# CleanDiffuserTeam/CleanDiffuser

Hardware: NVIDIA B200
Metric: sampled trajectories/sec (H=32, 100 DDPM steps) (higher is better)
Workload: dtype tf32 (fp32 activations and weights in HBM, tcgen05 kind::tf32, f32 accumulate)

## Files before the change

### __graft_entry__.py

```python
import os
import subprocess
import sys

ROOT = os.path.dirname(os.path.abspath(__file__))
CSRC = os.path.join(ROOT, "cleandiffuser_b200", "csrc")
LIB = os.path.join(CSRC, "libcds.so")
TC_PARTS = 8
HEADERS = ["common.cuh", "conv_simt.cuh", "conv_tc.cuh", "conv_ps.cuh", "ptx_sm100.cuh", "elementwise.cuh", "attention.cuh",
           os.path.join(ROOT, "include", "cds.h")]
OBJ_DIR = os.path.join(CSRC, "build")

NVCC_FLAGS = ["-gencode", "arch=compute_100a,code=sm_100a", "-O3", "-lineinfo", "-std=c++17",
              "-Xcompiler", "-fPIC", "-I" + os.path.join(ROOT, "include")]


def _units():
    units = [(os.path.join(OBJ_DIR, "cds_api.o"), os.path.join(CSRC, "cds_api.cu"), [])]
    for tf32 in (0, 1):
        for k in range(TC_PARTS):
            units.append((os.path.join(OBJ_DIR, f"conv_tc_inst_{k}_{'tf32' if tf32 else 'bf16'}.o"),
                          os.path.join(CSRC, "conv_tc_inst.cu"),
                          [f"-DCDS_TC_PART={k}", f"-DCDS_TC_PARTS={TC_PARTS}", f"-DCDS_TC_TF32={tf32}"]))
    units.append((os.path.join(OBJ_DIR, "conv_ps_inst.o"), os.path.join(CSRC, "conv_ps_inst.cu"), []))
    return units


def _newest_dep():
    deps = [f if os.path.isabs(f) else os.path.join(CSRC, f) for f in HEADERS]
    deps += [os.path.join(CSRC, f) for f in os.listdir(CSRC) if f.endswith((".cu", ".cuh"))]
    return max(os.path.getmtime(d) for d in deps if os.path.exists(d))


def build(force: bool = False) -> None:
    from concurrent.futures import ThreadPoolExecutor
    nvcc = os.environ.get("NVCC", "/usr/local/cuda/bin/nvcc")
    os.makedirs(OBJ_DIR, exist_ok=True)
    newest = _newest_dep()
    todo = [u for u in _units() if force or not os.path.exists(u[0]) or os.path.getmtime(u[0]) < newest]

    def compile_one(u):
        cmd = [nvcc] + NVCC_FLAGS + u[2] + ["-c", u[1], "-o", u[0]]
        print("[build]", " ".join(cmd), flush=True)
        r = subprocess.run(cmd, cwd=CSRC, capture_output=True, text=True)
        return u[0], r.returncode, r.stdout + r.stderr

    if todo:
        with ThreadPoolExecutor(max_workers=min(len(todo), os.cpu_count() or 1)) as ex:
            results = list(ex.map(compile_one, todo))
        for obj, rc, out in results:
            if rc != 0:
                raise RuntimeError(f"nvcc failed for {obj}:\n{out}")
    objs = [u[0] for u in _units()]
    if todo or not os.path.exists(LIB) or os.path.getmtime(LIB) < max(os.path.getmtime(o) for o in objs):
        cmd = [nvcc, "-gencode", "arch=compute_100a,code=sm_100a", "-shared", "-Xcompiler", "-fPIC"] + objs + ["-o", LIB]
        print("[build]", " ".join(cmd), flush=True)
        subprocess.run(cmd, check=True, cwd=CSRC)
    if ROOT not in sys.path:
        sys.path.insert(0, ROOT)
    import cleandiffuser_b200
    from cleandiffuser_b200.engine import cabi
    import ctypes
    lib = ctypes.CDLL(cabi.lib_path())
    missing = [s for s in cabi.EXPORTS if not hasattr(lib, s)]
    if missing:
        raise RuntimeError(f"libcds.so lacks symbols {missing}")
    print("[build] ok:", cabi.lib_path(), flush=True)


def smoke() -> None:
    if ROOT not in sys.path:
        sys.path.insert(0, ROOT)
    import torch
    from cleandiffuser_b200.diffusion import DiscreteDiffusionSDE
    from cleandiffuser_b200.engine import runtime
    from cleandiffuser_b200.nn_diffusion import JannerUNet1d
    from cleandiffuser_b200.testing import NoiseTape, load_synth
    import oracle.nets as onets
    import oracle.sampler as osamp

    assert torch.cuda.is_available(), "smoke() needs a CUDA device"
    os.environ["CDS_BACKEND"] = "cuda"
    dev = "cuda:0"
    B, H, D, T = 64, 32, 14, 10
    net = load_synth(JannerUNet1d(D, model_dim=32, emb_dim=32, kernel_size=5, dim_mult=[1, 2, 2, 2]), seed=0)
    sd = {k: v.clone() for k, v in net.state_dict().items()}
    mask = torch.zeros(H, D)
    mask[0, :11] = 1.
    agent = DiscreteDiffusionSDE(net, None, fix_mask=mask, predict_noise=False, diffusion_steps=T, device=dev)
    g = torch.Generator().manual_seed(1)
    prior = torch.zeros(B, H, D)
    prior[:, 0, :11] = torch.randn(B, 11, generator=g)

    fn = lambda x, t, c=None: onets.janner_unet(sd, x, t, c, emb_dim=32, kernel_size=5, n_stages=4)
    x_ref = None
    for math, tol_max, tol_mean in (("tf32", 2e-2, 2e-3), ("bf16", 0.2, 0.02), ("fp32", 2e-3, 2e-3)):
        os.environ["CDS_MATH"] = math
        before = runtime.STATS["engine_calls"]
        tape = NoiseTape() if x_ref is None else NoiseTape(tape.draws)
        with tape.active(), torch.no_grad():
            x_gpu, _ = agent.sample(prior.to(dev), solver="ddpm", n_samples=B, sample_steps=T, temperature=0.5)
        torch.cuda.synchronize()
        assert runtime.STATS["engine_calls"] == before + 1, "the CUDA engine did not run"
        if x_ref is None:
            with torch.no_grad():
                x_ref = osamp.sample_discrete(fn, prior, osamp.Tape([z.cpu().numpy() for z in tape.draws]), T=T, steps=T,
                                              solver="ddpm", temperature=0.5, fix_mask=mask[None], predict_noise=False)
        err = (x_gpu.cpu() - x_ref).abs()
        print(f"[smoke] JannerUNet1d B={B} H={H} d={D} DDPM {T} steps, math={math}: max|engine - oracle| = {err.max().item():.3e}, "
              f"mean = {err.mean().item():.3e}, launches={runtime.STATS['launches']}")
        assert err.max().item() < tol_max and err.mean().item() < tol_mean, (math, err.max().item(), err.mean().item())


if __name__ == "__main__":
    build()
    if len(sys.argv) > 1 and sys.argv[1] == "smoke":
        smoke()
```

### cleandiffuser_b200/csrc/cds_api.cu

```cuda
#include <cuda_runtime.h>

#include <cstdarg>
#include <cstdio>
#include <cstring>
#include <string>
#include <vector>

#include "cds.h"
#include "attention.cuh"
#include "conv_simt.cuh"
#include "conv_tc.cuh"
#include "conv_ps.cuh"
#include "attention_tma.cuh"
#include "linear_ln.cuh"
#include "elementwise.cuh"

namespace {

thread_local std::string g_err;

int fail(int code, const char* fmt, ...) {
  char buf[512];
  va_list ap;
  va_start(ap, fmt);
  vsnprintf(buf, sizeof buf, fmt, ap);
  va_end(ap);
  g_err = buf;
  return code;
}

#define CDS_CUDA(call)                                                                                  \
  do {                                                                                                  \
    cudaError_t e__ = (call);                                                                           \
    if (e__ != cudaSuccess) return fail(CDS_ERR_CUDA, "%s failed: %s", #call, cudaGetErrorString(e__)); \
  } while (0)

struct DeviceGuard {
  int prev = -1;
  cudaError_t err = cudaSuccess;
  explicit DeviceGuard(int device) {
    err = cudaGetDevice(&prev);
    if (err == cudaSuccess && prev != device) err = cudaSetDevice(device);
    else if (err == cudaSuccess) prev = -1;
  }
  ~DeviceGuard() { if (prev >= 0) cudaSetDevice(prev); }
};
#define CDS_ON_DEVICE(dev)                                                                                       \
  DeviceGuard guard__(dev);                                                                                      \
  if (guard__.err != cudaSuccess) return fail(CDS_ERR_CUDA, "cudaSetDevice(%d) failed: %s", (int)(dev), cudaGetErrorString(guard__.err))

struct Step {
  cds_op op;
  int conv_bn = 0;
  bool tc = false;
  cds::ConvTcLaunch tcl;
  int branch = 0;
  bool skip = false;
  bool ps = false;
  cds::ConvPsLaunch psl;
  cds::AttnTmaLaunch attl;
  bool fuse_ln = false;
  bool fused_into_prev = false;
  cds::LinLnLaunch lll;
};

int elementwise_grid(int64_t total, int sm_count) {
  int64_t blocks = (total + 255) / 256;
  int64_t cap = (int64_t)sm_count * 8;
  return (int)(blocks < cap ? (blocks > 0 ? blocks : 1) : cap);
}

int validate(const cds_op& op, Step* out) {
  out->op = op;
  out->branch = (op.flags & CDS_OPF_BRANCH_MASK) >> CDS_OPF_BRANCH_SHIFT;
  switch (op.kind) {
    case CDS_OP_CONV: {
      const cds_conv_op& c = op.u.conv;
      if (c.batch <= 0 || c.L_in <= 0 || c.L_out <= 0 || c.C_in <= 0 || c.C_out <= 0 || c.taps <= 0 ||
          c.stride <= 0 || c.phases <= 0)
        return fail(CDS_ERR_INVALID, "conv: non-positive geometry");
      if (!c.in || !c.w || !c.out) return fail(CDS_ERR_INVALID, "conv: null in/w/out");
      if (c.groups > 8) return fail(CDS_ERR_UNSUPPORTED, "conv: more than 8 GroupNorm groups");
      if (c.groups > 0 && (!c.gn_gamma || !c.gn_beta)) return fail(CDS_ERR_INVALID, "conv: GroupNorm without affine");
      if (c.res_w && (!c.res_in || c.res_C <= 0)) return fail(CDS_ERR_INVALID, "conv: shortcut conv without input");
      if (c.res_w && (c.stride != 1 || c.phases != 1)) return fail(CDS_ERR_INVALID, "conv: shortcut conv needs stride 1");
      if (c.math == CDS_MATH_BF16_TC || c.math == CDS_MATH_TF32_TC) {
        if (!cds::conv_tc_eligible(c))
          return fail(CDS_ERR_INVALID, "conv: op is not eligible for the tensor-core kernel (ask cds_conv_tc_supported)");
        if (cds::conv_ps_eligible(c)) {
          if (!cds::conv_ps_prepare(c, &out->psl))
            return fail(CDS_ERR_CUDA, "conv: cuTensorMapEncodeTiled failed (position-sliced, C_in=%d C_out=%d)", c.C_in, c.C_out);
          out->tc = out->ps = true;
          return CDS_OK;
        }
        if (!cds::conv_tc_prepare(c, &out->tcl))
          return fail(CDS_ERR_CUDA, "conv: cuTensorMapEncodeTiled failed (C_in=%d L=%d C_out=%d)", c.C_in, c.L_in, c.C_out);
        out->tc = true;
        return CDS_OK;
      }
      if (c.math != CDS_MATH_FP32) return fail(CDS_ERR_UNSUPPORTED, "conv: math mode %d unknown", c.math);
      if (c.sample_row_div > 1) return fail(CDS_ERR_UNSUPPORTED, "conv: sample_row_div needs the tensor-core kernel");
      out->conv_bn = cds::conv_simt_pick_bn(c);
      if (out->conv_bn == 0)
        return fail(CDS_ERR_UNSUPPORTED, "conv: GroupNorm tile does not fit (L_out=%d C_out=%d groups=%d)", c.L_out,
                    c.C_out, c.groups);
      return CDS_OK;
    }
    case CDS_OP_UPDATE: {
      const cds_update_op& u = op.u.update;
      if (u.batch <= 0 || u.row <= 0 || !u.x || !u.pred || !u.coef) return fail(CDS_ERR_INVALID, "update: bad arguments");
      if (u.mask && !u.prior) return fail(CDS_ERR_INVALID, "update: mask without prior");
      if (u.aux && !u.xhat_prev) return fail(CDS_ERR_INVALID, "update: aux history without xhat_prev");
      if (u.x_cast && (u.cast_C_in <= 0 || u.cast_C_out < u.cast_C_in || u.row % u.cast_C_in != 0))
        return fail(CDS_ERR_INVALID, "update: bad x_cast geometry");
      return CDS_OK;
    }
    case CDS_OP_LNMOD: {
      const cds_lnmod_op& l = op.u.lnmod;
      if (l.batch <= 0 || l.L <= 0 || l.C <= 0 || !l.in || !l.out || !l.shift || !l.scale)
        return fail(CDS_ERR_INVALID, "lnmod: bad arguments");
      return CDS_OK;
    }
    case CDS_OP_ATTN: {
      const cds_attn_op& a = op.u.attn;
      if (a.batch <= 0 || a.L <= 0 || a.heads <= 0 || a.C % a.heads != 0 || !a.qkv || !a.out)
        return fail(CDS_ERR_INVALID, "attn: bad arguments");
      int hd = a.C / a.heads;
      if (hd != 16 && hd != 32 && hd != 64) return fail(CDS_ERR_UNSUPPORTED, "attn: head_dim %d", hd);
      if ((size_t)a.L * hd * 8 > 200 * 1024) return fail(CDS_ERR_UNSUPPORTED, "attn: L=%d too long", a.L);
      if (a.qkv_dtype == CDS_BF16 && (hd != 32 || a.L > cds::kAttnMaxL || a.C % 8 != 0 || ((uintptr_t)a.qkv % 16) != 0))
        return fail(CDS_ERR_UNSUPPORTED, "attn: bf16 q/k/v needs head_dim 32, L <= %d, 16-byte aligned rows", cds::kAttnMaxL);
      if (cds::attention_tma_eligible(a) && !cds::attention_tma_prepare(a, &out->attl))
        return fail(CDS_ERR_CUDA, "attn: cuTensorMapEncodeTiled failed (L=%d C=%d)", a.L, a.C);
      return CDS_OK;
    }
    case CDS_OP_PREP: {
      const cds_prep_op& p = op.u.prep;
      if (p.batch <= 0 || p.row <= 0 || !p.x || !p.xin || !p.coef) return fail(CDS_ERR_INVALID, "prep: bad arguments");
      return CDS_OK;
    }
    case CDS_OP_CAST: {
      const cds_cast_op& k = op.u.cast;
      if (k.batch <= 0 || k.L <= 0 || k.C_in <= 0 || k.C_out < k.C_in || (k.C_out & 1) || !k.in || !k.out ||
          (k.out_dtype != CDS_F32 && k.out_dtype != CDS_BF16 && k.out_dtype != CDS_TF32))
        return fail(CDS_ERR_INVALID, "cast: bad arguments");
      return CDS_OK;
    }
    default:
      return fail(CDS_ERR_INVALID, "unknown operator kind %d", op.kind);
  }
}

int launch(const Step& s, const int* iter_ptr, int sm_count, cudaStream_t st, int* advance = nullptr, bool fused = false) {
  switch (s.op.kind) {
    case CDS_OP_CONV:
      if (fused && s.fuse_ln) CDS_CUDA(cds::linear_ln_launch(s.lll, iter_ptr, sm_count, st));
      else if (s.ps) CDS_CUDA(cds::conv_ps_launch(s.psl, iter_ptr, st));
      else if (s.tc) CDS_CUDA(cds::conv_tc_launch(s.tcl, iter_ptr, st));
      else CDS_CUDA(cds::conv_simt_launch(s.op.u.conv, s.conv_bn, iter_ptr, st));
      return CDS_OK;
    case CDS_OP_UPDATE: {
      const cds_update_op& u = s.op.u.update;
      cds::solver_update_kernel<<<elementwise_grid((int64_t)u.batch * u.row, sm_count), 256, 0, st>>>(u, iter_ptr, advance);
      CDS_CUDA(cudaGetLastError());
      return CDS_OK;
    }
    case CDS_OP_PREP: {
      const cds_prep_op& p = s.op.u.prep;
      cds::cm_prep_kernel<<<elementwise_grid((int64_t)p.batch * p.row, sm_count), 256, 0, st>>>(p, iter_ptr);
      CDS_CUDA(cudaGetLastError());
      return CDS_OK;
    }
    case CDS_OP_LNMOD: {
      const cds_lnmod_op& l = s.op.u.lnmod;
      int64_t rows = (int64_t)l.batch * l.L;
      int64_t blocks = (rows + 7) / 8;
      int64_t cap = (int64_t)sm_count * 8;
      cds::ln_modulate_kernel<<<(int)(blocks < cap ? blocks : cap), 256, 0, st>>>(l);
      CDS_CUDA(cudaGetLastError());
      return CDS_OK;
    }
    case CDS_OP_ATTN:
      if (s.attl.ok) CDS_CUDA(cds::attention_tma_launch(s.op.u.attn, s.attl, sm_count, st));
      else CDS_CUDA(cds::attention_launch(s.op.u.attn, st));
      return CDS_OK;
    case CDS_OP_CAST: {
      const cds_cast_op& k = s.op.u.cast;
      cds::cast_pad_kernel<<<elementwise_grid((int64_t)k.batch * k.L * (k.C_out / 2), sm_count), 256, 0, st>>>(k);
      CDS_CUDA(cudaGetLastError());
      return CDS_OK;
    }
  }
  return fail(CDS_ERR_INVALID, "unknown operator kind");
}

int preload_kernels() {
  cudaFuncAttributes a;
  CDS_CUDA(cudaFuncGetAttributes(&a, cds::conv_gemm_f32_kernel<32>));
  CDS_CUDA(cudaFuncGetAttributes(&a, cds::conv_gemm_f32_kernel<64>));
  CDS_CUDA(cudaFuncGetAttributes(&a, cds::conv_gemm_f32_kernel<128>));
  CDS_CUDA(cds::conv_tc_preload_all());
  CDS_CUDA(cds::conv_ps_preload_all());
  CDS_CUDA(cudaFuncGetAttributes(&a, cds::attention_f32_kernel<16>));
  CDS_CUDA(cudaFuncGetAttributes(&a, cds::attention_f32_kernel<32>));
  CDS_CUDA(cudaFuncGetAttributes(&a, cds::attention_f32_kernel<64>));
  CDS_CUDA(cudaFuncGetAttributes(&a, cds::attention_mma_hd32_kernel));
  CDS_CUDA(cudaFuncGetAttributes(&a, cds::attention_mma_tf32_hd32_kernel));
  CDS_CUDA(cds::attention_tma_preload_all());
  CDS_CUDA(cds::linear_ln_preload_all());
  CDS_CUDA(cudaFuncGetAttributes(&a, cds::solver_update_kernel));
  CDS_CUDA(cudaFuncGetAttributes(&a, cds::cm_prep_kernel));
  CDS_CUDA(cudaFuncGetAttributes(&a, cds::cast_pad_kernel));
  CDS_CUDA(cudaFuncGetAttributes(&a, cds::ln_modulate_kernel));
  CDS_CUDA(cudaFuncGetAttributes(&a, cds::set_iter_kernel));
  CDS_CUDA(cudaFuncGetAttributes(&a, cds::advance_iter_kernel));
  return CDS_OK;
}

}

namespace cds {
static long long* g_trace_buf = nullptr;
static int64_t g_trace_cap = 0;
static int g_trace_target = -1, g_trace_count = 0, g_trace_grid = 0;
long long* conv_tc_trace_hook(int grid) {
  if (!g_trace_buf) return nullptr;
  const int ord = g_trace_count++;
  if (ord != g_trace_target || (int64_t)grid * kTraceSlots > g_trace_cap) return nullptr;
  g_trace_grid = grid;
  return g_trace_buf;
}
}

struct cds_plan {
  int device = 0;
  int sm_count = 0;
  int n_iters = 0;
  bool finalized = false;
  std::vector<Step> steps;
  int* d_iter = nullptr;
  cudaStream_t cap_stream = nullptr;
  cudaGraph_t graph = nullptr;
  cudaGraphExec_t exec = nullptr;
  int multi = 0;
  int n_branches = 1;
  std::vector<cudaStream_t> side;
  cudaEvent_t ev_fork = nullptr;
  std::vector<cudaEvent_t> ev_join;
  cudaGraph_t graph_multi = nullptr;
  cudaGraphExec_t exec_multi = nullptr;
};

extern "C" {

int cds_version(void) { return CDS_ABI_VERSION; }
int cds_op_size(void) { return (int)sizeof(cds_op); }
const char* cds_last_error(void) { return g_err.c_str(); }

int cds_conv_tc_supported(const cds_conv_op* op) {
  if (!op) return 0;
  cds_conv_op c = *op;
  if (c.math != CDS_MATH_TF32_TC) c.math = CDS_MATH_BF16_TC;
  return cds::conv_tc_eligible(c) ? 1 : 0;
}

int cds_device_sm_count(int device) {
  int n = 0;
  if (cudaDeviceGetAttribute(&n, cudaDevAttrMultiProcessorCount, device) != cudaSuccess) return -1;
  return n;
}

int cds_plan_create(int device, cds_plan** out) {
  if (!out) return fail(CDS_ERR_INVALID, "plan_create: null out");
  int n_dev = 0;
  CDS_CUDA(cudaGetDeviceCount(&n_dev));
  if (device < 0 || device >= n_dev) return fail(CDS_ERR_INVALID, "plan_create: device %d of %d", device, n_dev);
  cds_plan* p = new cds_plan();
  p->device = device;
  p->sm_count = cds_device_sm_count(device);
  *out = p;
  return CDS_OK;
}

int cds_plan_destroy(cds_plan* p) {
  if (!p) return CDS_OK;
  DeviceGuard guard(p->device);
  if (p->exec) cudaGraphExecDestroy(p->exec);
  if (p->graph) cudaGraphDestroy(p->graph);
  if (p->exec_multi) cudaGraphExecDestroy(p->exec_multi);
  if (p->graph_multi) cudaGraphDestroy(p->graph_multi);
  if (p->cap_stream) cudaStreamDestroy(p->cap_stream);
  for (cudaStream_t s : p->side) cudaStreamDestroy(s);
  if (p->ev_fork) cudaEventDestroy(p->ev_fork);
  for (cudaEvent_t e : p->ev_join) cudaEventDestroy(e);
  if (p->d_iter) cudaFree(p->d_iter);
  delete p;
  return CDS_OK;
}

int cds_plan_append(cds_plan* p, const cds_op* ops, int32_t n_ops) {
  if (!p || (!ops && n_ops > 0)) return fail(CDS_ERR_INVALID, "plan_append: null argument");
  if (p->finalized) return fail(CDS_ERR_STATE, "plan_append after finalize");
  for (int i = 0; i < n_ops; ++i) {
    Step s;
    int rc = validate(ops[i], &s);
    if (rc != CDS_OK) {
      std::string inner = g_err;
      return fail(rc, "op %d: %s", (int)p->steps.size(), inner.c_str());
    }
    p->steps.push_back(s);
  }
  return CDS_OK;
}

int cds_plan_finalize(cds_plan* p, int32_t n_iters) {
  if (!p) return fail(CDS_ERR_INVALID, "plan_finalize: null plan");
  if (p->finalized) return fail(CDS_ERR_STATE, "plan already finalized");
  if (n_iters <= 0 || p->steps.empty()) return fail(CDS_ERR_INVALID, "plan_finalize: empty program");
  CDS_ON_DEVICE(p->device);
  { int rc = preload_kernels(); if (rc != CDS_OK) return rc; }
  CDS_CUDA(cudaMalloc(&p->d_iter, 2 * sizeof(int)));
  CDS_CUDA(cudaMemset(p->d_iter, 0, 2 * sizeof(int)));
  CDS_CUDA(cudaStreamCreateWithFlags(&p->cap_stream, cudaStreamNonBlocking));
  p->n_iters = n_iters;
  for (const Step& s : p->steps) if (s.branch + 1 > p->n_branches) p->n_branches = s.branch + 1;
  if (p->n_branches > 1) {
    CDS_CUDA(cudaEventCreateWithFlags(&p->ev_fork, cudaEventDisableTiming));
    for (int b = 1; b < p->n_branches; ++b) {
      cudaStream_t s; cudaEvent_t e;
      CDS_CUDA(cudaStreamCreateWithFlags(&s, cudaStreamNonBlocking));
      CDS_CUDA(cudaEventCreateWithFlags(&e, cudaEventDisableTiming));
      p->side.push_back(s); p->ev_join.push_back(e);
    }
    for (Step& s : p->steps) if (s.tc && !s.ps) s.tcl.max_ctas_per_sm = 1;
  }
  if (p->n_branches == 1) {
    for (size_t i = 0; i + 1 < p->steps.size(); ++i) {
      Step& a = p->steps[i];
      Step& b = p->steps[i + 1];
      if (a.op.kind != CDS_OP_CONV || b.op.kind != CDS_OP_LNMOD || !a.tc || a.ps) continue;
      if ((a.op.flags & CDS_OPF_ONCE) || (b.op.flags & CDS_OPF_ONCE)) continue;
      if (!cds::linear_ln_eligible(a.op.u.conv, b.op.u.lnmod)) continue;
      if (!cds::linear_ln_prepare(a.op.u.conv, b.op.u.lnmod, &a.lll)) continue;
      a.fuse_ln = true;
      b.fused_into_prev = true;
    }
  }
  p->finalized = true;
  return CDS_OK;
}

static bool advance_fused(const cds_plan* p) {
  if (p->n_branches > 1) return false;
  for (int i = (int)p->steps.size() - 1; i >= 0; --i)
    if (!(p->steps[i].op.flags & CDS_OPF_ONCE)) return p->steps[i].op.kind == CDS_OP_UPDATE;
  return false;
}

static int enqueue_once(cds_plan* p, cudaStream_t st) {
  for (const Step& s : p->steps) {
    if (!(s.op.flags & CDS_OPF_ONCE)) continue;
    int rc = launch(s, p->d_iter, p->sm_count, st);
    if (rc != CDS_OK) return rc;
  }
  return CDS_OK;
}

static int enqueue_iteration(cds_plan* p, cudaStream_t st) {
  const bool fused = advance_fused(p);
  if (p->n_branches == 1) {
    int last = -1;
    for (int i = 0; i < (int)p->steps.size(); ++i) if (!(p->steps[i].op.flags & CDS_OPF_ONCE)) last = i;
    for (int i = 0; i < (int)p->steps.size(); ++i) {
      const Step& s = p->steps[i];
      if ((s.op.flags & CDS_OPF_ONCE) || s.skip || s.fused_into_prev) continue;
      int rc = launch(s, p->d_iter, p->sm_count, st, (fused && i == last) ? p->d_iter : nullptr, true);
      if (rc != CDS_OK) return rc;
    }
  } else {
    CDS_CUDA(cudaEventRecord(p->ev_fork, st));
    for (cudaStream_t s : p->side) CDS_CUDA(cudaStreamWaitEvent(s, p->ev_fork, 0));
    std::vector<std::vector<int>> per(p->n_branches);
    for (int i = 0; i < (int)p->steps.size(); ++i) {
      const Step& s = p->steps[i];
      if (!(s.op.flags & CDS_OPF_ONCE) && !s.skip) per[s.branch].push_back(i);
    }
    for (size_t k = 0;; ++k) {
      bool any = false;
      for (int b = 0; b < p->n_branches; ++b) {
        if (k >= per[b].size()) continue;
        any = true;
        int rc = launch(p->steps[per[b][k]], p->d_iter, p->sm_count, b == 0 ? st : p->side[b - 1], nullptr);
        if (rc != CDS_OK) return rc;
      }
      if (!any) break;
    }
    for (int b = 1; b < p->n_branches; ++b) {
      CDS_CUDA(cudaEventRecord(p->ev_join[b - 1], p->side[b - 1]));
      CDS_CUDA(cudaStreamWaitEvent(st, p->ev_join[b - 1], 0));
    }
  }
  if (!fused) {
    cds::advance_iter_kernel<<<1, 1, 0, st>>>(p->d_iter);
    CDS_CUDA(cudaGetLastError());
  }
  return CDS_OK;
}

int cds_plan_run(cds_plan* p, int32_t first, int32_t count, void* stream, int32_t use_graph) {
  if (!p || !p->finalized) return fail(CDS_ERR_STATE, "plan_run before finalize");
  if (first < 0 || count < 0 || first + count > p->n_iters)
    return fail(CDS_ERR_INVALID, "plan_run: iterations [%d, %d) outside [0, %d)", first, first + count, p->n_iters);
  cudaStream_t st = reinterpret_cast<cudaStream_t>(stream);
  CDS_ON_DEVICE(p->device);
  if (use_graph && !p->exec) {
    CDS_CUDA(cudaStreamBeginCapture(p->cap_stream, cudaStreamCaptureModeThreadLocal));
    int rc = enqueue_iteration(p, p->cap_stream);
    cudaError_t e = cudaStreamEndCapture(p->cap_stream, &p->graph);
    if (rc != CDS_OK) return rc;
    if (e != cudaSuccess) return fail(CDS_ERR_CUDA, "graph capture failed: %s", cudaGetErrorString(e));
    CDS_CUDA(cudaGraphInstantiate(&p->exec, p->graph, 0));
    const char* gi = getenv("CDS_GRAPH_ITERS");
    p->multi = gi ? atoi(gi) : 10;
    if (p->multi > 1 && p->multi <= p->n_iters) {
      CDS_CUDA(cudaStreamBeginCapture(p->cap_stream, cudaStreamCaptureModeThreadLocal));
      int rc2 = CDS_OK;
      for (int k = 0; k < p->multi && rc2 == CDS_OK; ++k) rc2 = enqueue_iteration(p, p->cap_stream);
      cudaError_t e2 = cudaStreamEndCapture(p->cap_stream, &p->graph_multi);
      if (rc2 != CDS_OK) return rc2;
      if (e2 != cudaSuccess) return fail(CDS_ERR_CUDA, "graph capture (x%d) failed: %s", p->multi, cudaGetErrorString(e2));
      CDS_CUDA(cudaGraphInstantiate(&p->exec_multi, p->graph_multi, 0));
    } else {
      p->multi = 0;
    }
  }
  cds::set_iter_kernel<<<1, 1, 0, st>>>(p->d_iter, first);
  CDS_CUDA(cudaGetLastError());
  { int rc = enqueue_once(p, st); if (rc != CDS_OK) return rc; }
  for (int i = 0; i < count; ++i) {
    if (use_graph && p->exec_multi && count - i >= p->multi) {
      CDS_CUDA(cudaGraphLaunch(p->exec_multi, st));
      i += p->multi - 1;
    } else if (use_graph) {
      CDS_CUDA(cudaGraphLaunch(p->exec, st));
    } else {
      int rc = enqueue_iteration(p, st);
      if (rc != CDS_OK) return rc;
    }
  }
  return CDS_OK;
}

int cds_plan_run_range(cds_plan* p, int32_t iter, int32_t op_first, int32_t op_count, void* stream) {
  if (!p || !p->finalized) return fail(CDS_ERR_STATE, "plan_run_range before finalize");
  if (iter < 0 || iter >= p->n_iters) return fail(CDS_ERR_INVALID, "plan_run_range: iteration %d outside [0, %d)", iter, p->n_iters);
  if (op_first < 0 || op_count < 0 || op_first + op_count > (int)p->steps.size())
    return fail(CDS_ERR_INVALID, "plan_run_range: operators [%d, %d) outside [0, %d)", op_first, op_first + op_count, (int)p->steps.size());
  if (p->n_branches > 1) return fail(CDS_ERR_UNSUPPORTED, "plan_run_range: programs with parallel branches run whole iterations only");
  cudaStream_t st = reinterpret_cast<cudaStream_t>(stream);
  CDS_ON_DEVICE(p->device);
  cds::set_iter_kernel<<<1, 1, 0, st>>>(p->d_iter, iter);
  CDS_CUDA(cudaGetLastError());
  for (int i = op_first; i < op_first + op_count; ++i) {
    const Step& s = p->steps[i];
    if ((s.op.flags & CDS_OPF_ONCE) || s.skip) continue;
    if (s.fused_into_prev && i > op_first) continue;
    const bool both = s.fuse_ln && i + 1 < op_first + op_count;
    int rc = launch(s, p->d_iter, p->sm_count, st, nullptr, both);
    if (rc != CDS_OK) return rc;
  }
  return CDS_OK;
}

int cds_plan_profile(cds_plan* p, int32_t iter, void* stream, float* ms_per_op, int32_t n_ops) {
  if (!p || !p->finalized) return fail(CDS_ERR_STATE, "plan_profile before finalize");
  if (!ms_per_op || n_ops != (int)p->steps.size()) return fail(CDS_ERR_INVALID, "plan_profile: n_ops != %d", (int)p->steps.size());
  if (iter < 0 || iter >= p->n_iters) return fail(CDS_ERR_INVALID, "plan_profile: bad iteration");
  cudaStream_t st = reinterpret_cast<cudaStream_t>(stream);
  CDS_ON_DEVICE(p->device);
  std::vector<cudaEvent_t> ev(2 * n_ops);
  for (auto& e : ev) CDS_CUDA(cudaEventCreate(&e));
  cds::set_iter_kernel<<<1, 1, 0, st>>>(p->d_iter, iter);
  for (int pass = 0; pass < 2; ++pass) {
    for (int i = 0; i < n_ops; ++i) {
      const bool once = (p->steps[i].op.flags & CDS_OPF_ONCE) != 0;
      if (once != (pass == 0)) continue;
      CDS_CUDA(cudaEventRecord(ev[2 * i], st));
      if (!p->steps[i].skip && !p->steps[i].fused_into_prev) {
        int rc = launch(p->steps[i], p->d_iter, p->sm_count, st, nullptr, true);
        if (rc != CDS_OK) return rc;
      }
      CDS_CUDA(cudaEventRecord(ev[2 * i + 1], st));
    }
  }
  CDS_CUDA(cudaStreamSynchronize(st));
  for (int i = 0; i < n_ops; ++i) CDS_CUDA(cudaEventElapsedTime(&ms_per_op[i], ev[2 * i], ev[2 * i + 1]));
  for (auto& e : ev) cudaEventDestroy(e);
  return CDS_OK;
}

int cds_plan_launches_per_iter(const cds_plan* p) {
  if (!p) return 0;
  int n = advance_fused(p) ? 0 : 1;
  for (const Step& s : p->steps) if (!(s.op.flags & CDS_OPF_ONCE) && !s.skip && !s.fused_into_prev) ++n;
  return n;
}

int cds_debug_trace(void* device_buffer, int64_t capacity_entries, int32_t target_launch) {
  cds::g_trace_buf = reinterpret_cast<long long*>(device_buffer);
  cds::g_trace_cap = capacity_entries;
  cds::g_trace_target = target_launch;
  cds::g_trace_count = 0;
  int g = cds::g_trace_grid;
  cds::g_trace_grid = 0;
  return g;
}

int cds_run_op(int device, const cds_op* op, int32_t iter, void* stream) {
  if (!op) return fail(CDS_ERR_INVALID, "run_op: null op");
  CDS_ON_DEVICE(device);
  Step s;
  int rc = validate(*op, &s);
  if (rc != CDS_OK) return rc;
  cudaStream_t st = reinterpret_cast<cudaStream_t>(stream);
  int* d_iter = nullptr;
  CDS_CUDA(cudaMallocAsync(&d_iter, sizeof(int), st));
  cds::set_iter_kernel<<<1, 1, 0, st>>>(d_iter, iter);
  rc = launch(s, d_iter, cds_device_sm_count(device), st);
  cudaFreeAsync(d_iter, st);
  return rc;
}

}
```

Measured before the change: 67880.

## Fuse both tensor-core convolutions of a residual block into one persistent kernel

Adds a warp-specialized tcgen05 kernel that runs conv1+GroupNorm+Mish, keeps the hidden activation in shared memory, then runs conv2+GroupNorm+Mish plus the identity or 1x1-conv residual, all in one launch. The plan finalizer pairs consecutive TC conv steps when the intermediate buffer is read by no other step. The aim is to cut one launch per residual block and the HBM round trip of the intermediate. In exchange it adds a large new kernel with its own smem/TMEM planning and a more complex pipeline. It can be turned off with CDS_FUSE_RESBLOCK=0.

```diff
diff --git a/__graft_entry__.py b/__graft_entry__.py
--- a/__graft_entry__.py
+++ b/__graft_entry__.py
@@ -6,7 +6,7 @@
 CSRC = os.path.join(ROOT, "cleandiffuser_b200", "csrc")
 LIB = os.path.join(CSRC, "libcds.so")
 TC_PARTS = 8
-HEADERS = ["common.cuh", "conv_simt.cuh", "conv_tc.cuh", "conv_ps.cuh", "ptx_sm100.cuh", "elementwise.cuh", "attention.cuh",
+HEADERS = ["common.cuh", "conv_simt.cuh", "conv_tc.cuh", "conv_ps.cuh", "resblock_tc.cuh", "ptx_sm100.cuh", "elementwise.cuh", "attention.cuh",
            os.path.join(ROOT, "include", "cds.h")]
 OBJ_DIR = os.path.join(CSRC, "build")
 
@@ -22,6 +22,7 @@
                           os.path.join(CSRC, "conv_tc_inst.cu"),
                           [f"-DCDS_TC_PART={k}", f"-DCDS_TC_PARTS={TC_PARTS}", f"-DCDS_TC_TF32={tf32}"]))
     units.append((os.path.join(OBJ_DIR, "conv_ps_inst.o"), os.path.join(CSRC, "conv_ps_inst.cu"), []))
+    units.append((os.path.join(OBJ_DIR, "resblock_tc_inst.o"), os.path.join(CSRC, "resblock_tc_inst.cu"), []))
     return units
 
 
diff --git a/cleandiffuser_b200/csrc/cds_api.cu b/cleandiffuser_b200/csrc/cds_api.cu
--- a/cleandiffuser_b200/csrc/cds_api.cu
+++ b/cleandiffuser_b200/csrc/cds_api.cu
@@ -13,6 +13,7 @@
 #include "conv_ps.cuh"
 #include "attention_tma.cuh"
 #include "linear_ln.cuh"
+#include "resblock_tc.cuh"
 #include "elementwise.cuh"
 
 namespace {
@@ -62,7 +63,24 @@
   bool fuse_ln = false;
   bool fused_into_prev = false;
   cds::LinLnLaunch lll;
+  bool fuse_rb = false;
+  cds::ResblockLaunch rbl;
 };
+
+bool step_reads(const Step& s, const void* lo, const void* hi) {
+  auto in = [&](const void* q) { return q && q >= lo && q < hi; };
+  const cds_op& o = s.op;
+  switch (o.kind) {
+    case CDS_OP_CONV: return in(o.u.conv.in) || in(o.u.conv.res) || in(o.u.conv.res_in);
+    case CDS_OP_UPDATE: return in(o.u.update.x) || in(o.u.update.pred) || in(o.u.update.pred_uncond) || in(o.u.update.prior) ||
+                               in(o.u.update.xhat_prev) || in(o.u.update.aux);
+    case CDS_OP_LNMOD: return in(o.u.lnmod.in);
+    case CDS_OP_ATTN: return in(o.u.attn.qkv);
+    case CDS_OP_PREP: return in(o.u.prep.x);
+    case CDS_OP_CAST: return in(o.u.cast.in);
+  }
+  return true;
+}
 
 int elementwise_grid(int64_t total, int sm_count) {
   int64_t blocks = (total + 255) / 256;
@@ -155,6 +173,7 @@
   switch (s.op.kind) {
     case CDS_OP_CONV:
       if (fused && s.fuse_ln) CDS_CUDA(cds::linear_ln_launch(s.lll, iter_ptr, sm_count, st));
+      else if (fused && s.fuse_rb) CDS_CUDA(cds::resblock_launch(s.rbl, iter_ptr, sm_count, st));
       else if (s.ps) CDS_CUDA(cds::conv_ps_launch(s.psl, iter_ptr, st));
       else if (s.tc) CDS_CUDA(cds::conv_tc_launch(s.tcl, iter_ptr, st));
       else CDS_CUDA(cds::conv_simt_launch(s.op.u.conv, s.conv_bn, iter_ptr, st));
@@ -208,6 +227,7 @@
   CDS_CUDA(cudaFuncGetAttributes(&a, cds::attention_mma_tf32_hd32_kernel));
   CDS_CUDA(cds::attention_tma_preload_all());
   CDS_CUDA(cds::linear_ln_preload_all());
+  CDS_CUDA(cds::resblock_preload_all());
   CDS_CUDA(cudaFuncGetAttributes(&a, cds::solver_update_kernel));
   CDS_CUDA(cudaFuncGetAttributes(&a, cds::cm_prep_kernel));
   CDS_CUDA(cudaFuncGetAttributes(&a, cds::cast_pad_kernel));
@@ -344,6 +364,26 @@
       if (!cds::linear_ln_prepare(a.op.u.conv, b.op.u.lnmod, &a.lll)) continue;
       a.fuse_ln = true;
       b.fused_into_prev = true;
+    }
+  }
+  const char* frb = getenv("CDS_FUSE_RESBLOCK");
+  if (p->n_branches == 1 && !(frb && frb[0] == '0')) {
+    for (size_t i = 0; i + 1 < p->steps.size(); ++i) {
+      Step& a = p->steps[i];
+      Step& b = p->steps[i + 1];
+      if (a.op.kind != CDS_OP_CONV || b.op.kind != CDS_OP_CONV || !a.tc || a.ps || !b.tc || b.ps) continue;
+      if ((a.op.flags & CDS_OPF_ONCE) || (b.op.flags & CDS_OPF_ONCE)) continue;
+      if (a.fuse_ln || a.fused_into_prev || b.fuse_ln || b.fused_into_prev) continue;
+      const cds_conv_op& c = a.op.u.conv;
+      const char* lo = reinterpret_cast<const char*>(c.out);
+      const char* hi = lo + 4 * ((int64_t)(c.batch - 1) * c.out_bstride + (int64_t)(c.L_out - 1) * c.out_lstride + c.C_out);
+      bool shared = false;
+      for (size_t k = 0; k < p->steps.size() && !shared; ++k)
+        if (k != i + 1 && step_reads(p->steps[k], lo, hi)) shared = true;
+      if (shared || !cds::resblock_prepare(c, b.op.u.conv, &a.rbl)) continue;
+      a.fuse_rb = true;
+      b.fused_into_prev = true;
+      ++i;
     }
   }
   p->finalized = true;
@@ -465,7 +505,7 @@
     const Step& s = p->steps[i];
     if ((s.op.flags & CDS_OPF_ONCE) || s.skip) continue;
     if (s.fused_into_prev && i > op_first) continue;
-    const bool both = s.fuse_ln && i + 1 < op_first + op_count;
+    const bool both = (s.fuse_ln || s.fuse_rb) && i + 1 < op_first + op_count;
     int rc = launch(s, p->d_iter, p->sm_count, st, nullptr, both);
     if (rc != CDS_OK) return rc;
   }
diff --git a/cleandiffuser_b200/csrc/resblock_tc.cuh b/cleandiffuser_b200/csrc/resblock_tc.cuh
--- /dev/null
+++ b/cleandiffuser_b200/csrc/resblock_tc.cuh
@@ -0,0 +1,485 @@
+#pragma once
+#include <cuda.h>
+
+#include <cstdio>
+#include <cstdlib>
+
+#include "common.cuh"
+#include "ptx_sm100.cuh"
+#include "conv_tc.cuh"
+
+namespace cds {
+
+constexpr int kRbThreads = 320;
+constexpr int kRbEpiThreads = 256;
+constexpr int kRbMaxStages = 16;
+constexpr int kRbRowBytes = 128;
+
+struct ResblockParams {
+  CUtensorMap tm_x;
+  CUtensorMap tm_w1, tm_w2, tm_wr;
+  CUtensorMap tm_out;
+  int batch, L, T, num_tiles;
+  int kc1;
+  int xbufs, stages, resident;
+  const float* b1; int64_t b1_stride;
+  const float* b2; int64_t b2_stride;
+  const float* shift1; int64_t shift1_stride;
+  const float *g1, *be1, *g2, *be2; float eps1, eps2;
+  const float* res_bias;
+};
+
+template <int N>
+struct RbCfg {
+  static constexpr int kKc2 = N / 32;
+  static constexpr int kStageBytes = N * kRbRowBytes;
+  static constexpr int kMinBlocks = N <= 64 ? 2 : 1;
+  static constexpr int kNH = N / 2;
+  static constexpr int kCPG = N / 8;
+  static constexpr int kStaticBytes = 8 * 2048 + 8 * N * 4 + 2 * 4 * 8 * 16 * 8 + 2048;
+};
+template <int N, bool RES>
+struct RbTmem {
+  static constexpr int kNeed = N * (RES ? 3 : 2);
+  static constexpr uint32_t kCols = kNeed <= 64 ? 64 : (kNeed <= 128 ? 128 : (kNeed <= 256 ? 256 : 512));
+};
+
+template <int N, bool RES>
+__global__ void __launch_bounds__(kRbThreads, RbCfg<N>::kMinBlocks)
+resblock_tc_kernel(const __grid_constant__ ResblockParams p, const int* __restrict__ iter_ptr) {
+  using Cfg = RbCfg<N>;
+  constexpr int KC2 = Cfg::kKc2, NH = Cfg::kNH, CPG = Cfg::kCPG, GPT = NH / CPG;
+  constexpr uint32_t kTmemCols = RbTmem<N, RES>::kCols;
+  extern __shared__ uint8_t smem_raw[];
+  __shared__ __align__(8) uint64_t full_bar[kRbMaxStages], empty_bar[kRbMaxStages];
+  __shared__ __align__(8) uint64_t x_full[2], x_empty[2], acc1_full, h_full, acc2_full;
+  __shared__ uint32_t tmem_base_holder;
+  __shared__ __align__(16) float s_col[8][N];
+  __shared__ __align__(1024) uint8_t s_stage[kRbEpiThreads / 32][2048];
+  __shared__ __align__(16) float2 s_red[2][4][8][16];
+
+  const int warp = threadIdx.x >> 5, lane = threadIdx.x & 31;
+  const uint32_t smem_base = (ptx::smem_u32(smem_raw) + 1023u) & ~1023u;
+  uint8_t* smem_al = smem_raw + (smem_base - ptx::smem_u32(smem_raw));
+  const int T = p.T, RX = 128 + 4 * p.T;
+  const uint32_t chunk_bytes = (uint32_t)RX * kRbRowBytes;
+  const uint32_t x_off = 0;
+  const uint32_t h_off = x_off + (uint32_t)(p.xbufs * p.kc1) * chunk_bytes;
+  const uint32_t w_off = h_off + (uint32_t)KC2 * chunk_bytes;
+  const int n_w1 = 5 * p.kc1, n_w2 = 5 * KC2, n_w = n_w1 + n_w2 + (RES ? p.kc1 : 0);
+  const int n_my = p.num_tiles > (int)blockIdx.x ? (p.num_tiles - 1 - (int)blockIdx.x) / (int)gridDim.x + 1 : 0;
+
+  if (threadIdx.x == 0) {
+    for (int s = 0; s < p.stages; ++s) { ptx::mbar_init(&full_bar[s], 1); ptx::mbar_init(&empty_bar[s], 1); }
+    for (int i = 0; i < 2; ++i) { ptx::mbar_init(&x_full[i], 1); ptx::mbar_init(&x_empty[i], kRbEpiThreads / 32); }
+    ptx::mbar_init(&acc1_full, 1); ptx::mbar_init(&acc2_full, 1); ptx::mbar_init(&h_full, kRbEpiThreads / 32);
+    ptx::fence_barrier_init();
+  }
+  if (warp == 8 && lane == 0) {
+    ptx::prefetch_tensormap(&p.tm_x); ptx::prefetch_tensormap(&p.tm_w1); ptx::prefetch_tensormap(&p.tm_w2);
+    if (RES) ptx::prefetch_tensormap(&p.tm_wr);
+    ptx::prefetch_tensormap(&p.tm_out);
+  }
+  if (warp == 9) ptx::tmem_alloc<kTmemCols>(&tmem_base_holder);
+  ptx::tc_fence_before_sync();
+  __syncthreads();
+  ptx::tc_fence_after_sync();
+  const uint32_t tmem_base = tmem_base_holder;
+  if (threadIdx.x == 0) ptx::grid_dep_launch_dependents();
+
+  if (warp == 8) {
+    if (ptx::elect_one()) {
+      auto load_w = [&](int kb, int s) {
+        uint8_t* dst = smem_al + w_off + (uint32_t)s * Cfg::kStageBytes;
+        ptx::mbar_expect_tx(&full_bar[s], Cfg::kStageBytes);
+        if (kb < n_w1) ptx::tma_load_2d(dst, &p.tm_w1, &full_bar[s], (kb % p.kc1) * 32, (kb / p.kc1) * N);
+        else if (kb < n_w1 + n_w2) { const int k2 = kb - n_w1; ptx::tma_load_2d(dst, &p.tm_w2, &full_bar[s], (k2 % KC2) * 32, (k2 / KC2) * N); }
+        else ptx::tma_load_2d(dst, &p.tm_wr, &full_bar[s], (kb - n_w1 - n_w2) * 32, 0);
+      };
+      auto load_x = [&](int it_) {
+        if (it_ >= n_my) return;
+        const int tile = (int)blockIdx.x + it_ * (int)gridDim.x;
+        const int xb = it_ % p.xbufs;
+        const uint32_t use = (uint32_t)(it_ / p.xbufs);
+        ptx::mbar_wait(&x_empty[xb], (use & 1) ^ 1);
+        ptx::mbar_expect_tx(&x_full[xb], (uint32_t)p.kc1 * chunk_bytes);
+        uint8_t* dst = smem_al + x_off + (uint32_t)(xb * p.kc1) * chunk_bytes;
+        for (int ck = 0; ck < p.kc1; ++ck)
+          ptx::tma_load_3d(dst + ck * chunk_bytes, &p.tm_x, &x_full[xb], ck * 32, tile * T, -2);
+      };
+      int pre = 0;
+      if (n_my > 0) {
+        pre = n_w < p.stages ? n_w : p.stages;
+        for (int kb = 0; kb < pre; ++kb) load_w(kb, kb);
+      }
+      ptx::grid_dep_wait();
+      if (p.xbufs == 2) load_x(0);
+      int ring = 0;
+      for (int it = 0; it < n_my; ++it) {
+        for (int kb = 0; kb < n_w; ++kb) {
+        if (kb == (p.xbufs == 2 ? n_w1 : 0)) load_x(it + p.xbufs - 1);
+          if (p.resident) continue;
+          const int s = ring % p.stages;
+          const uint32_t ph = (uint32_t)(ring / p.stages) & 1;
+          if (ring >= pre) { ptx::mbar_wait(&empty_bar[s], ph ^ 1); load_w(kb, s); }
+          ++ring;
+        }
+      }
+    }
+  } else if (warp == 9) {
+    if (ptx::elect_one() && n_my > 0) {
+      constexpr uint32_t idesc = ptx::make_idesc_tf32(128, N);
+      const uint32_t acc1 = tmem_base, acc2 = tmem_base + (uint32_t)N, accr = tmem_base + 2u * (uint32_t)N;
+      int ring = 0;
+      auto step = [&](uint32_t a_addr, uint32_t d, bool first) {
+        const int s = p.resident ? ring % n_w : ring % p.stages;
+        const uint32_t ph = p.resident ? 0u : (uint32_t)(ring / p.stages) & 1;
+        ptx::mbar_wait(&full_bar[s], ph);
+        ptx::tc_fence_after_sync();
+        const uint64_t da = ptx::make_kmajor_desc<kRbRowBytes>(a_addr);
+        const uint64_t db = ptx::make_kmajor_desc<kRbRowBytes>(smem_base + w_off + (uint32_t)s * Cfg::kStageBytes);
+#pragma unroll
+        for (int k = 0; k < 4; ++k) ptx::umma_tf32(d, da + (uint64_t)(2 * k), db + (uint64_t)(2 * k), idesc, (first && k == 0) ? 0u : 1u);
+        if (!p.resident) ptx::umma_commit(&empty_bar[s]);
+        ++ring;
+      };
+      auto conv1 = [&](int it_) {
+        const int xb = it_ % p.xbufs;
+        ptx::mbar_wait(&x_full[xb], (uint32_t)(it_ / p.xbufs) & 1);
+        ptx::tc_fence_after_sync();
+        const uint32_t xa = smem_base + x_off + (uint32_t)(xb * p.kc1) * chunk_bytes;
+        for (int j = 0; j < 5; ++j)
+          for (int ck = 0; ck < p.kc1; ++ck) step(xa + ck * chunk_bytes + (uint32_t)(j * T * kRbRowBytes), acc1, j == 0 && ck == 0);
+        ptx::umma_commit(&acc1_full);
+      };
+      conv1(0);
+      for (int it = 0; it < n_my; ++it) {
+        ptx::mbar_wait(&h_full, (uint32_t)it & 1);
+        ptx::tc_fence_after_sync();
+        const uint32_t ha = smem_base + h_off;
+        for (int j = 0; j < 5; ++j)
+          for (int cc = 0; cc < KC2; ++cc) step(ha + cc * chunk_bytes + (uint32_t)(j * T * kRbRowBytes), acc2, j == 0 && cc == 0);
+        if constexpr (RES) {
+          const uint32_t xa = smem_base + x_off + (uint32_t)((it % p.xbufs) * p.kc1) * chunk_bytes + (uint32_t)(2 * T * kRbRowBytes);
+          for (int ck = 0; ck < p.kc1; ++ck) step(xa + ck * chunk_bytes, accr, ck == 0);
+        }
+        ptx::umma_commit(&acc2_full);
+        if (it + 1 < n_my) conv1(it + 1);
+      }
+    }
+  } else {
+    ptx::grid_dep_wait();
+    const int iter = iter_ptr ? *iter_ptr : 0;
+    for (int n = threadIdx.x; n < N; n += kRbEpiThreads) {
+      s_col[0][n] = __ldg(p.b1 + (int64_t)iter * p.b1_stride + n);
+      s_col[1][n] = __ldg(p.g1 + n);
+      s_col[2][n] = __ldg(p.be1 + n);
+      s_col[3][n] = p.shift1 ? __ldg(p.shift1 + (int64_t)iter * p.shift1_stride + n) : 0.f;
+      s_col[4][n] = __ldg(p.b2 + (int64_t)iter * p.b2_stride + n);
+      s_col[5][n] = __ldg(p.g2 + n);
+      s_col[6][n] = __ldg(p.be2 + n);
+      s_col[7][n] = (RES && p.res_bias) ? __ldg(p.res_bias + n) : 0.f;
+    }
+    for (int i = threadIdx.x; i < KC2 * 4 * T * 8; i += kRbEpiThreads) {
+      const int cc = i / (4 * T * 8), r = (i / 8) % (4 * T), u = i % 8;
+      const int row = r < 2 * T ? r : 128 + r;
+      *reinterpret_cast<float4*>(smem_al + h_off + cc * chunk_bytes + row * kRbRowBytes + u * 16) = make_float4(0.f, 0.f, 0.f, 0.f);
+    }
+    ptx::fence_proxy_async();
+    ptx::named_bar_sync(1, kRbEpiThreads);
+
+    const int q = warp & 3, half = warp >> 2;
+    const int m = 32 * q + lane;
+    const int t = lane & (T - 1);
+    const int col0 = half * NH;
+    const uint32_t t_lane = tmem_base + ((uint32_t)(32 * q) << 16);
+    const int hrow = 2 * T + m;
+    const uint32_t row_off = (uint32_t)hrow * kRbRowBytes;
+    const int sw = hrow & 7;
+    const float inv_cnt = 1.f / (float)(p.L * CPG);
+    uint8_t* const stg = &s_stage[warp][0];
+    uint8_t* const stg_row = stg + lane * 64;
+
+    auto gn = [&](int e, uint32_t acc, const float* bias, float (&v)[NH], float eps, float (&ga)[GPT], float (&gc)[GPT]) {
+      constexpr int W = NH < 32 ? NH : 32;
+#pragma unroll
+      for (int c = 0; c < NH; c += W) ptx::tmem_ld<W>(t_lane + acc + (uint32_t)(col0 + c), *reinterpret_cast<float(*)[W]>(&v[c]));
+      float s1[GPT], s2[GPT];
+#pragma unroll
+      for (int g = 0; g < GPT; ++g) { s1[g] = 0.f; s2[g] = 0.f; }
+#pragma unroll
+      for (int k = 0; k < NH / 4; ++k) {
+        const float4 bb = reinterpret_cast<const float4*>(bias + col0)[k];
+        const int g = (4 * k) / CPG;
+        const float x0 = (v[4 * k] += bb.x), x1 = (v[4 * k + 1] += bb.y), x2 = (v[4 * k + 2] += bb.z), x3 = (v[4 * k + 3] += bb.w);
+        s1[g] += (x0 + x1) + (x2 + x3);
+        s2[g] = fmaf(x0, x0, s2[g]); s2[g] = fmaf(x1, x1, s2[g]); s2[g] = fmaf(x2, x2, s2[g]); s2[g] = fmaf(x3, x3, s2[g]);
+      }
+      for (int off = T; off < 32; off <<= 1) {
+#pragma unroll
+        for (int g = 0; g < GPT; ++g) {
+          s1[g] += __shfl_xor_sync(0xffffffffu, s1[g], off);
+          s2[g] += __shfl_xor_sync(0xffffffffu, s2[g], off);
+        }
+      }
+      if (lane < T) {
+#pragma unroll
+        for (int g = 0; g < GPT; ++g) s_red[e][q][half * GPT + g][lane] = make_float2(s1[g], s2[g]);
+      }
+      ptx::named_bar_sync(2 + half, 128);
+#pragma unroll
+      for (int g = 0; g < GPT; ++g) {
+        float S1 = 0.f, S2 = 0.f;
+#pragma unroll
+        for (int qq = 0; qq < 4; ++qq) { const float2 r = s_red[e][qq][half * GPT + g][t]; S1 += r.x; S2 += r.y; }
+        const float mean = S1 * inv_cnt;
+        const float rstd = rsqrt_ftz(fmaxf(fmaf(S2, inv_cnt, -mean * mean), 0.f) + eps);
+        ga[g] = rstd; gc[g] = -mean * rstd;
+      }
+    };
+
+    for (int it = 0; it < n_my; ++it) {
+      const int tile = (int)blockIdx.x + it * (int)gridDim.x;
+      const int xb = it % p.xbufs;
+      const uint8_t* const xrow = smem_al + x_off + (uint32_t)(xb * p.kc1) * chunk_bytes + row_off;
+      {
+        ptx::mbar_wait(&acc1_full, (uint32_t)it & 1);
+        ptx::tc_fence_after_sync();
+        float v[NH], ga[GPT], gc[GPT];
+        gn(0, 0u, &s_col[0][0], v, p.eps1, ga, gc);
+#pragma unroll
+        for (int k = 0; k < NH / 4; ++k) {
+          const int n = col0 + 4 * k, g = (4 * k) / CPG;
+          const float4 gm = reinterpret_cast<const float4*>(&s_col[1][n])[0];
+          const float4 be = reinterpret_cast<const float4*>(&s_col[2][n])[0];
+          const float4 sh = reinterpret_cast<const float4*>(&s_col[3][n])[0];
+          const float o0 = mish_fma(fmaf(fmaf(v[4 * k + 0], ga[g], gc[g]), gm.x, be.x), sh.x);
+          const float o1 = mish_fma(fmaf(fmaf(v[4 * k + 1], ga[g], gc[g]), gm.y, be.y), sh.y);
+          const float o2 = mish_fma(fmaf(fmaf(v[4 * k + 2], ga[g], gc[g]), gm.z, be.z), sh.z);
+          const float o3 = mish_fma(fmaf(fmaf(v[4 * k + 3], ga[g], gc[g]), gm.w, be.w), sh.w);
+          const int u = (n & 31) >> 2;
+          *reinterpret_cast<float4*>(smem_al + h_off + (uint32_t)(n >> 5) * chunk_bytes + row_off + ((u ^ sw) << 4)) =
+              make_float4(round_tf32(o0), round_tf32(o1), round_tf32(o2), round_tf32(o3));
+        }
+        ptx::fence_proxy_async();
+        ptx::tc_fence_before_sync();
+        __syncwarp();
+        if (lane == 0) ptx::mbar_arrive(&h_full);
+      }
+      {
+        ptx::mbar_wait(&acc2_full, (uint32_t)it & 1);
+        ptx::tc_fence_after_sync();
+        if (!RES) ptx::mbar_wait(&x_full[xb], (uint32_t)(it / p.xbufs) & 1);
+        float v[NH], ga[GPT], gc[GPT];
+        gn(1, (uint32_t)N, &s_col[4][0], v, p.eps2, ga, gc);
+#pragma unroll
+        for (int h = 0; h < NH / 16; ++h) {
+          const int n0 = col0 + 16 * h;
+          if (lane == 0) ptx::bulk_wait_group_read<0>();
+          __syncwarp();
+#pragma unroll
+          for (int k = 0; k < 4; ++k) {
+            const float4 gm = reinterpret_cast<const float4*>(&s_col[5][n0])[k];
+            const float4 be = reinterpret_cast<const float4*>(&s_col[6][n0])[k];
+            const int g = (16 * h + 4 * k) / CPG;
+            const float* vv = &v[16 * h + 4 * k];
+            float addv[4];
+            if constexpr (RES) {
+              ptx::tmem_ld<4>(t_lane + 2u * (uint32_t)N + (uint32_t)(n0 + 4 * k), addv);
+              const float4 rb = reinterpret_cast<const float4*>(&s_col[7][n0])[k];
+              addv[0] = addv[0] + rb.x; addv[1] = addv[1] + rb.y; addv[2] = addv[2] + rb.z; addv[3] = addv[3] + rb.w;
+            } else {
+              const int u = ((n0 & 31) >> 2) + k;
+              const float4 r = *reinterpret_cast<const float4*>(xrow + (uint32_t)(n0 >> 5) * chunk_bytes + ((u ^ sw) << 4));
+              addv[0] = r.x; addv[1] = r.y; addv[2] = r.z; addv[3] = r.w;
+            }
+            const float o0 = mish_fma(fmaf(fmaf(vv[0], ga[g], gc[g]), gm.x, be.x), addv[0]);
+            const float o1 = mish_fma(fmaf(fmaf(vv[1], ga[g], gc[g]), gm.y, be.y), addv[1]);
+            const float o2 = mish_fma(fmaf(fmaf(vv[2], ga[g], gc[g]), gm.z, be.z), addv[2]);
+            const float o3 = mish_fma(fmaf(fmaf(vv[3], ga[g], gc[g]), gm.w, be.w), addv[3]);
+            *reinterpret_cast<float4*>(stg_row + ((k ^ ((lane >> 1) & 3)) << 4)) =
+                make_float4(round_tf32(o0), round_tf32(o1), round_tf32(o2), round_tf32(o3));
+          }
+          ptx::fence_proxy_async();
+          __syncwarp();
+          if (lane == 0) {
+            ptx::tma_store_3d(&p.tm_out, stg, n0, tile * T, (32 * q) / T);
+            ptx::bulk_commit_group();
+          }
+        }
+        ptx::tc_fence_before_sync();
+        __syncwarp();
+        if (lane == 0) ptx::mbar_arrive(&x_empty[xb]);
+      }
+    }
+    if (lane == 0) ptx::bulk_wait_group<0>();
+  }
+  __syncthreads();
+  if (warp == 9) {
+    ptx::tc_fence_after_sync();
+    ptx::tmem_dealloc<kTmemCols>(tmem_base);
+  }
+}
+
+struct ResblockLaunch {
+  ResblockParams prm;
+  int n = 0;
+  bool res = false;
+  int ctas_per_sm = 1;
+  int smem = 0;
+  dim3 grid;
+};
+
+inline bool resblock_plan(int L, int C_in, int C_out, bool res, int* xbufs, int* stages, int* resident, int* ctas, int* smem) {
+  if (L != 8 && L != 16 && L != 32) return false;
+  if (C_in % 32 || (C_out != 32 && C_out != 64 && C_out != 128)) return false;
+  const int T = 128 / L, RX = 128 + 4 * T, chunk = RX * kRbRowBytes;
+  const int kc1 = C_in / 32, kc2 = C_out / 32;
+  const int stage = C_out * kRbRowBytes;
+  const int n_w = 5 * kc1 + 5 * kc2 + (res ? kc1 : 0);
+  const int static_b = 8 * 2048 + 8 * C_out * 4 + 2 * 4 * 8 * 16 * 8 + 2048;
+  const int tmem = C_out * (res ? 3 : 2);
+  for (int c = 2; c >= 1; --c) {
+    if (c == 2 && (C_out > 64 || tmem > 256)) continue;
+    const int budget = (228 * 1024) / c - 1024 - static_b - 1024;
+    for (int xb = 2; xb >= 1; --xb) {
+      const int fixed = (xb * kc1 + kc2) * chunk;
+      if (fixed + 3 * stage > budget) continue;
+      int s = (budget - fixed) / stage;
+      int res_w = 0;
+      if (n_w <= kRbMaxStages && s >= n_w) { s = n_w; res_w = 1; }
+      else s = s > 8 ? 8 : s;
+      *xbufs = xb; *stages = s; *resident = res_w; *ctas = c;
+      *smem = fixed + s * stage + 1024;
+      return true;
+    }
+  }
+  return false;
+}
+
+inline bool resblock_encode_out(CUtensorMap* m, void* base, int C, int batch, int L, int64_t bstride, int lstride, int T) {
+  PFN_encodeTiled enc = get_encode_tiled();
+  if (!enc) return false;
+  cuuint64_t gdim[3] = {(cuuint64_t)C, (cuuint64_t)batch, (cuuint64_t)L};
+  cuuint64_t gstr[2] = {(cuuint64_t)bstride * 4, (cuuint64_t)lstride * 4};
+  cuuint32_t bx[3] = {16u, (cuuint32_t)T, (cuuint32_t)(32 / T)};
+  cuuint32_t es[3] = {1u, 1u, 1u};
+  return enc(m, CU_TENSOR_MAP_DATA_TYPE_FLOAT32, 3, base, gdim, gstr, bx, es, CU_TENSOR_MAP_INTERLEAVE_NONE, CU_TENSOR_MAP_SWIZZLE_64B,
+             CU_TENSOR_MAP_L2_PROMOTION_NONE, CU_TENSOR_MAP_FLOAT_OOB_FILL_NONE) == CUDA_SUCCESS;
+}
+
+inline bool resblock_prepare(const cds_conv_op& a, const cds_conv_op& b, ResblockLaunch* out) {
+  auto k5 = [](const cds_conv_op& c) {
+    return c.math == CDS_MATH_TF32_TC && c.stride == 1 && c.phases == 1 && c.taps == 5 && c.pad == 2 && c.groups == 8 &&
+           c.act == CDS_ACT_MISH && c.L_in == c.L_out && c.in_batch_mod == 0 && c.sample_row_div <= 1 && !c.scale.step &&
+           !c.scale.sample && !c.bias.sample && !c.shift.sample && c.bias.step;
+  };
+  if (!k5(a) || !k5(b)) return false;
+  const int L = a.L_out, C_in = a.C_in, C = a.C_out;
+  if (b.L_out != L || b.batch != a.batch || b.C_in != C || b.C_out != C) return false;
+  if (b.in != a.out || b.in_bstride != a.out_bstride || b.in_lstride != a.out_lstride) return false;
+  if (a.res || a.res_w || b.shift.step) return false;
+  if (a.out_dtype != CDS_TF32 || b.out_dtype != CDS_TF32 || (a.in_dtype != CDS_F32 && a.in_dtype != CDS_TF32)) return false;
+  const bool ident = b.res == a.in && !b.res_w && b.res_bstride == a.in_bstride && b.res_lstride == a.in_lstride &&
+                     b.res_batch_mod == 0 && C_in == C && b.res_dtype != CDS_BF16;
+  const bool conv = b.res_w && !b.res && b.res_in == a.in && b.res_in_bstride == a.in_bstride && b.res_in_lstride == a.in_lstride &&
+                    b.res_C == C_in && b.res_batch_mod == 0 && b.res_in_dtype != CDS_BF16;
+  if (!ident && !conv) return false;
+  auto al16 = [](const void* ptr, int64_t bs, int64_t ls) { return ((uintptr_t)ptr % 16) == 0 && (bs * 4) % 16 == 0 && (ls * 4) % 16 == 0; };
+  if (!al16(a.in, a.in_bstride, a.in_lstride) || !al16(b.out, b.out_bstride, b.out_lstride)) return false;
+  ResblockLaunch& R = *out;
+  memset(&R.prm, 0, sizeof(R.prm));
+  ResblockParams& p = R.prm;
+  if (!resblock_plan(L, C_in, C, conv, &p.xbufs, &p.stages, &p.resident, &R.ctas_per_sm, &R.smem)) return false;
+  const int T = 128 / L;
+  {
+    uint64_t dims[3] = {(uint64_t)C_in, (uint64_t)a.batch, (uint64_t)L};
+    uint64_t str[2] = {(uint64_t)a.in_bstride, (uint64_t)a.in_lstride};
+    uint32_t box[3] = {32u, (uint32_t)T, (uint32_t)(L + 4)};
+    if (!encode_act_map(&p.tm_x, a.in, 3, dims, str, box, 64, true)) return false;
+  }
+  {
+    uint64_t d1[2] = {(uint64_t)C_in, (uint64_t)5 * C}, s1[1] = {(uint64_t)C_in};
+    uint64_t d2[2] = {(uint64_t)C, (uint64_t)5 * C}, s2[1] = {(uint64_t)C};
+    uint32_t box[2] = {32u, (uint32_t)C};
+    if (!encode_act_map(&p.tm_w1, a.w, 2, d1, s1, box, 64, true)) return false;
+    if (!encode_act_map(&p.tm_w2, b.w, 2, d2, s2, box, 64, true)) return false;
+    if (conv) {
+      uint64_t dr[2] = {(uint64_t)C_in, (uint64_t)C}, sr[1] = {(uint64_t)C_in};
+      if (!encode_act_map(&p.tm_wr, b.res_w, 2, dr, sr, box, 64, true)) return false;
+    }
+  }
+  if (!resblock_encode_out(&p.tm_out, b.out, C, b.batch, L, b.out_bstride, b.out_lstride, T)) return false;
+  p.batch = a.batch; p.L = L; p.T = T;
+  p.num_tiles = (a.batch + T - 1) / T;
+  p.kc1 = C_in / 32;
+  p.b1 = a.bias.step; p.b1_stride = a.bias.step_stride;
+  p.b2 = b.bias.step; p.b2_stride = b.bias.step_stride;
+  p.shift1 = a.shift.step; p.shift1_stride = a.shift.step_stride;
+  p.g1 = a.gn_gamma; p.be1 = a.gn_beta; p.eps1 = a.gn_eps;
+  p.g2 = b.gn_gamma; p.be2 = b.gn_beta; p.eps2 = b.gn_eps;
+  p.res_bias = conv ? b.res_bias : nullptr;
+  R.n = C; R.res = conv;
+  R.grid = dim3((unsigned)p.num_tiles);
+  return true;
+}
+
+template <int N, bool RES>
+cudaError_t resblock_launch_t(const ResblockLaunch& R, const int* iter_ptr, int sm_count, cudaStream_t st) {
+  static bool attr = false;
+  static bool pdl = true;
+  if (!attr) {
+    cudaError_t e = cudaFuncSetAttribute(resblock_tc_kernel<N, RES>, cudaFuncAttributeMaxDynamicSharedMemorySize,
+                                         227 * 1024 - RbCfg<N>::kStaticBytes);
+    if (e != cudaSuccess) return e;
+    e = cudaFuncSetAttribute(resblock_tc_kernel<N, RES>, cudaFuncAttributePreferredSharedMemoryCarveout, cudaSharedmemCarveoutMaxShared);
+    if (e != cudaSuccess) return e;
+    const char* pdl_env = getenv("CDS_PDL");
+    pdl = !(pdl_env && pdl_env[0] == '0');
+    attr = true;
+  }
+  const unsigned cap = (unsigned)(R.ctas_per_sm * sm_count);
+  cudaLaunchConfig_t cfg = {};
+  cfg.gridDim = dim3(R.grid.x < cap ? R.grid.x : cap); cfg.blockDim = dim3(kRbThreads); cfg.dynamicSmemBytes = (size_t)R.smem;
+  cfg.stream = st;
+  cudaLaunchAttribute at[1];
+  at[0].id = cudaLaunchAttributeProgrammaticStreamSerialization; at[0].val.programmaticStreamSerializationAllowed = 1;
+  cfg.attrs = at; cfg.numAttrs = pdl ? 1 : 0;
+  return cudaLaunchKernelEx(&cfg, resblock_tc_kernel<N, RES>, R.prm, iter_ptr);
+}
+template <int N, bool RES>
+cudaError_t resblock_preload_t() {
+  cudaFuncAttributes a;
+  return cudaFuncGetAttributes(&a, resblock_tc_kernel<N, RES>);
+}
+
+#define CDS_RB_VARIANTS(X) X(32) X(64) X(128)
+
+#ifndef CDS_RB_INSTANTIATE
+#define CDS_RB_EXTERN(N_)                                                                                              \
+  extern template cudaError_t resblock_launch_t<N_, false>(const ResblockLaunch&, const int*, int, cudaStream_t);     \
+  extern template cudaError_t resblock_launch_t<N_, true>(const ResblockLaunch&, const int*, int, cudaStream_t);      \
+  extern template cudaError_t resblock_preload_t<N_, false>();                                                         \
+  extern template cudaError_t resblock_preload_t<N_, true>();
+CDS_RB_VARIANTS(CDS_RB_EXTERN)
+#undef CDS_RB_EXTERN
+
+inline cudaError_t resblock_launch(const ResblockLaunch& R, const int* iter_ptr, int sm_count, cudaStream_t st) {
+#define CDS_RB_CASE(N_) \
+  if (R.n == N_) return R.res ? resblock_launch_t<N_, true>(R, iter_ptr, sm_count, st) : resblock_launch_t<N_, false>(R, iter_ptr, sm_count, st);
+  CDS_RB_VARIANTS(CDS_RB_CASE)
+#undef CDS_RB_CASE
+  return cudaErrorInvalidValue;
+}
+inline cudaError_t resblock_preload_all() {
+  cudaError_t e;
+#define CDS_RB_PRE(N_)                                                          \
+  if ((e = resblock_preload_t<N_, false>()) != cudaSuccess) return e;           \
+  if ((e = resblock_preload_t<N_, true>()) != cudaSuccess) return e;
+  CDS_RB_VARIANTS(CDS_RB_PRE)
+#undef CDS_RB_PRE
+  return cudaSuccess;
+}
+#endif
+
+}
diff --git a/cleandiffuser_b200/csrc/resblock_tc_inst.cu b/cleandiffuser_b200/csrc/resblock_tc_inst.cu
--- /dev/null
+++ b/cleandiffuser_b200/csrc/resblock_tc_inst.cu
@@ -0,0 +1,11 @@
+#define CDS_RB_INSTANTIATE
+#include "resblock_tc.cuh"
+
+namespace cds {
+#define CDS_RB_INST(N_)                                                                                        \
+  template cudaError_t resblock_launch_t<N_, false>(const ResblockLaunch&, const int*, int, cudaStream_t);    \
+  template cudaError_t resblock_launch_t<N_, true>(const ResblockLaunch&, const int*, int, cudaStream_t);     \
+  template cudaError_t resblock_preload_t<N_, false>();                                                        \
+  template cudaError_t resblock_preload_t<N_, true>();
+CDS_RB_VARIANTS(CDS_RB_INST)
+}
```

Result: slower. 63400, median of 6 (-6.6%).
